# Wil-Lee/NN_BVH

Measured on AMD Instinct MI355X. Metric: Mray/s (closest-hit + any-hit), higher is better.
Workload: dtype f32; 1 GPU; crown, 1000x1400: one wavefront pass of 8 spp per step (8 spp per GPU-film) — primary, bounce-1 and bounce-2 closest-hit, shadow any-hit towards the light quads (batches pre-generated, hence independent: ONE launch; the dependent form is dependent_step), rays in --ray-order tile (a caller-side order the reference's integrator does not form: ray_order_probe), RecordShadowRayResult + RGBFilm::AddSam; sample_sets=4, geometry=procedural stand-in for crown (3548192 tris; data/crown.npz absent), tree=sah, triangles=3548192, nodes=7032259, rays_primary=11200000, rays_bounce=7410327, rays_bounce2=4392209, parallelism=tile-sharded x1, BVH replicated, film all-gather after the pass

## Files before the change

### nn_bvh_amd/aggregate.py

```python
import ctypes

import numpy as np

from . import _lib
from ._lib import HIT_DTYPE, NODE_DTYPE, PRIM_DTYPE, RAY_DTYPE, NNBVHError, check, ptr

SPLIT_METHODS = {"sah": 0, "hlbvh": 1, "middle": 2, "equal": 3}


def make_prims(tri_indices=None, patch_indices=None):
    nt = 0 if tri_indices is None else len(tri_indices)
    npch = 0 if patch_indices is None else len(patch_indices)
    prims = np.zeros(nt + npch, PRIM_DTYPE)
    prims["id"] = np.arange(nt + npch, dtype=np.int32)
    if nt:
        prims["kind"][:nt] = 0
        prims["v"][:nt, :3] = np.asarray(tri_indices, np.int32).reshape(nt, 3)
    if npch:
        prims["kind"][nt:] = 1
        prims["v"][nt:] = np.asarray(patch_indices, np.int32).reshape(npch, 4)
    return prims


def make_rays(o, d, tmax=np.inf, time=0.0):
# ... 206 lines not shown
                self._h = L.nnbvh_scene_create_instanced_animated(
                    ptr(self.nodes), len(self.nodes), int(n_top_nodes), ptr(self.ordered_prims),
                    len(self.ordered_prims), ptr(self.verts), len(self.verts), ptr(self.instances),
                    len(self.instances), ptr(self.animated), self.device)
            else:
                self._h = L.nnbvh_scene_create_instanced(
                    ptr(self.nodes), len(self.nodes), int(n_top_nodes), ptr(self.ordered_prims),
                    len(self.ordered_prims), ptr(self.verts), len(self.verts), ptr(self.instances),
                    len(self.instances), self.device)
        elif prim_alpha is not None:
            self.normals = None if normals is None else np.ascontiguousarray(normals, np.float32).reshape(-1, 3)
            self.prim_alpha = np.ascontiguousarray(prim_alpha, np.float32).reshape(-1)
            self.uvs = None if uvs is None else np.ascontiguousarray(uvs, np.float32).reshape(-1, 2)
            assert len(self.prim_alpha) == len(self.ordered_prims)
            assert self.normals is None or len(self.normals) == len(self.verts)
            assert self.uvs is None or len(self.uvs) == len(self.verts)
            self._h = L.nnbvh_scene_create_with_attributes(
                ptr(self.nodes), len(self.nodes), ptr(self.ordered_prims), len(self.ordered_prims), ptr(self.verts),
                ptr(self.normals) if self.normals is not None else None,
                ptr(self.uvs) if self.uvs is not None else None, ptr(self.prim_alpha), len(self.verts), self.device)
        elif normals is not None:
            self.normals = np.ascontiguousarray(normals, np.float32).reshape(-1, 3)
            assert len(self.normals) == len(self.verts)
            self._h = L.nnbvh_scene_create_with_normals(ptr(self.nodes), len(self.nodes), ptr(self.ordered_prims),
                                                        len(self.ordered_prims), ptr(self.verts), ptr(self.normals),
                                                        len(self.verts), self.device)
        else:
            self._h = L.nnbvh_scene_create(ptr(self.nodes), len(self.nodes), ptr(self.ordered_prims),
                                           len(self.ordered_prims), ptr(self.verts), len(self.verts),
                                           self.device)
        if not self._h:
            raise NNBVHError("nnbvh_scene_create: " + _lib.last_error())
        self._read_info()

    def close(self):
        if getattr(self, "_h", None):
            _lib.lib().nnbvh_scene_destroy(self._h)
            self._h = None

    def __del__(self):
        try:
            self.close()
        except Exception:
            pass

    def set_option(self, key, value):
        check(_lib.lib().nnbvh_scene_set_option(self._h, key.encode(), int(value)),
              f"set_option({key})")

    def sched_stats(self, reset=True):
        out = np.zeros(16, np.uint64)
        check(_lib.lib().nnbvh_scene_sched_stats(self._h, ptr(out), int(reset)), "sched_stats")
        return dict(zip(("int_trips", "int_lanes", "prim_trips", "prim_lanes", "refill_trips",
                         "refill_lanes", "i_nint", "i_nprim", "i_nidle", "spare0", "int_cycles",
                         "prim_cycles", "refill_cycles", "spare1", "int_steps", "int_step_lanes"),
                        (int(x) for x in out)))

    def Bounds(self):
        out = np.zeros(6, np.float32)
        check(_lib.lib().nnbvh_scene_bounds(self._h, ptr(out)), "nnbvh_scene_bounds")
        return out[:3].copy(), out[3:].copy()

    def Intersect(self, rays, out=None):
        rays = np.ascontiguousarray(rays, RAY_DTYPE)
        hits = np.zeros(len(rays), HIT_DTYPE) if out is None else out
        assert hits.dtype == HIT_DTYPE and len(hits) == len(rays) and hits.flags.c_contiguous
        check(_lib.lib().nnbvh_intersect_closest(self._h, ptr(rays), len(rays), ptr(hits)),
              "nnbvh_intersect_closest")
        return hits

    def IntersectP(self, rays, counts=False):
        rays = np.ascontiguousarray(rays, RAY_DTYPE)
        occ = np.zeros(len(rays), np.uint8)
        if counts:
            vis = np.zeros(len(rays), np.int32)
            tst = np.zeros(len(rays), np.int32)
            check(_lib.lib().nnbvh_intersect_any(self._h, ptr(rays), len(rays), ptr(occ),
                                                 ptr(vis), ptr(tst)), "nnbvh_intersect_any")
            return occ, vis, tst
        check(_lib.lib().nnbvh_intersect_any(self._h, ptr(rays), len(rays), ptr(occ), None, None),
              "nnbvh_intersect_any")
        return occ

    def intersect_device(self, d_rays, d_hits, n, stream=0):
        check(_lib.lib().nnbvh_intersect_closest_device(self._h, d_rays, n, d_hits, stream),
              "nnbvh_intersect_closest_device")

    def trace_batches_device(self, batches, stream=0):
        arr = np.zeros(len(batches), _lib.BATCH_DTYPE)
        for i, b in enumerate(batches):
            arr[i]["kind"] = {"closest": 0, "any": 1}[b[0]]
            arr[i]["d_rays"], arr[i]["n"], arr[i]["d_out"] = b[1], b[2], b[3]
            if len(b) > 4:
                arr[i]["d_nodes_visited"], arr[i]["d_prim_tests"] = b[4] or 0, b[5] or 0
        check(_lib.lib().nnbvh_trace_batches_device(self._h, ptr(arr), len(arr), stream),
              "nnbvh_trace_batches_device")

    def trace_batches_candidates_device(self, batches, candidates, stream=0):
        assert len(candidates) == len(batches)
        arr = np.zeros(len(batches), _lib.BATCH_DTYPE)
        for i, b in enumerate(batches):
            arr[i]["kind"] = {"closest": 0, "any": 1}[b[0]]
            arr[i]["d_rays"], arr[i]["n"], arr[i]["d_out"] = b[1], b[2], b[3]
            if len(b) > 4:
                arr[i]["d_nodes_visited"], arr[i]["d_prim_tests"] = b[4] or 0, b[5] or 0
        cs = (_lib.HostCandidates * max(len(batches), 1))()
        for i, c in enumerate(candidates):
            if c is not None:
# ... 121 lines not shown
```

### nn_bvh_amd/csrc/bvh_capi.cpp

```cpp
#include <algorithm>
#include <cmath>
#include <cstring>
#include <limits>
#include <vector>

#include "bvh_build_gpu.h"
#include "capi_internal.h"

namespace nnbvh {

static thread_local std::string g_error;
void set_error(const std::string &msg) { g_error = msg; }

}

using namespace nnbvh;

static bool validate_tree(const nnbvh_linear_node *nodes, int root, int n_tree, const nnbvh_prim *prims,
                          int n_prims, bool allow_instances, std::vector<uint8_t> &covered,
                          std::vector<uint8_t> &leaf_last, int *depth_out) {
    if (n_tree < 1) {
        set_error("scene_create: tree has no nodes");
        return false;
    }
// ... 653 lines not shown
        return NNBVH_ERR_ARG;
    }
    std::memset(out, 0, 16 * sizeof(uint64_t));
    if (!s->d_stats) return NNBVH_OK;
    DeviceGuard guard(s->device);
    if (!guard.ok) return NNBVH_ERR_DEVICE;
    if (!hip_ok(hipDeviceSynchronize(), "scene_sched_stats") ||
        !hip_ok(hipMemcpy(out, s->d_stats, 16 * sizeof(uint64_t), hipMemcpyDeviceToHost),
                "scene_sched_stats"))
        return NNBVH_ERR_DEVICE;
    if (reset) (void)hipMemset(s->d_stats, 0, 16 * sizeof(unsigned long long));
    return NNBVH_OK;
}

int nnbvh_scene_set_option(nnbvh_scene *s, const char *key, int value) {
    if (!s || !key) {
        set_error("set_option: null argument");
        return NNBVH_ERR_ARG;
    }
    std::lock_guard<std::mutex> lock(s->mu);
    std::string k(key);
    if (k == "stack_window") {
        if (value != 4 && value != 8 && value != 16) {
            set_error("set_option: stack_window must be 4, 8 or 16");
            return NNBVH_ERR_ARG;
        }
        s->window = value;
    } else if (k == "blocks_per_cu") {
        if (value < 0 || value > 8) {
            set_error("set_option: blocks_per_cu must be 0..8");
            return NNBVH_ERR_ARG;
        }
        s->blocks_per_cu = value;
    } else if (k == "int_repeat") {
        if (value < 1 || value > 16) {
            set_error("set_option: int_repeat must be 1..16");
            return NNBVH_ERR_ARG;
        }
        s->int_repeat = value;
    } else if (k == "host_chunk") {
        if (value < 1024) {
            set_error("set_option: host_chunk must be at least 1024 rays");
            return NNBVH_ERR_ARG;
        }
        s->host_chunk = value;
    } else if (k == "prim_repeat") {
        if (value < 1 || value > 16) {
            set_error("set_option: prim_repeat must be 1..16");
            return NNBVH_ERR_ARG;
        }
        s->prim_repeat = value;
    } else if (k == "fused_batches") {
        s->fused_batches = value ? 1 : 0;
    } else if (k == "xcd_queues") {
        s->xcd_queues = value ? 1 : 0;
    } else if (k == "prim_weight") {
        if (value < 1 || value > 64) {
            set_error("set_option: prim_weight must be 1..64");
            return NNBVH_ERR_ARG;
        }
        s->prim_weight = value;
    } else if (k == "refill_weight") {
        if (value < 1 || value > 64) {
            set_error("set_option: refill_weight must be 1..64");
            return NNBVH_ERR_ARG;
        }
        s->refill_weight = value;
    } else {
        set_error("set_option: unknown key");
        return NNBVH_ERR_ARG;
    }
    return NNBVH_OK;
}

}

Workspace *nnbvh::workspace_for(nnbvh_scene *s, hipStream_t stream) {
    auto it = s->workspaces.find(stream);
    if (it != s->workspaces.end()) return &it->second;
    Workspace w;
    const size_t spill_bytes = (size_t)std::max(s->depth - 2, 1) * (size_t)s->max_grid_threads * sizeof(uint2);
    if (!hip_ok(hipMalloc((void **)&w.queue, kMaxFusedBatches * kMaxQueues * kQueueStrideWords * sizeof(unsigned)),
                "hipMalloc(queue)"))
        return nullptr;
    if (!hip_ok(hipMalloc((void **)&w.spill, spill_bytes), "hipMalloc(spill)")) {
        (void)hipFree(w.queue);
        return nullptr;
    }
    return &(s->workspaces[stream] = w);
}
```

### nn_bvh_amd/csrc/bvh_trace.h

```cpp
#pragma once
#include <hip/hip_runtime.h>
#include <stdint.h>

#include "../../include/nnbvh.h"
#include "nnbvh_internal.h"

namespace nnbvh {

constexpr int kBlockThreads = 256;
constexpr int kMaxQueues = 8;
constexpr int kQueueStrideWords = 32;
constexpr int kMaxFusedBatches = 4;
constexpr int kFusedIndexBits = 28;

struct TraceParams {
    const float4 *wide;
    const float4 *prims;
    float rootMin[3], rootMax[3];
    int rootRef;
    const nnbvh_ray *rays;
    nnbvh_hit *hits;
    uint8_t *occluded;
    int32_t *visitedOut;
    int32_t *testsOut;
    long n;
    const int32_t *nDev;
    unsigned *queue;
    int nQueues;
    int primWeight;
    int refillWeight;
    int hasHostPrims;
    int intRepeat;
    int primRepeat;
    int fits32;
    unsigned long long *stats;
    uint2 *spill;
    const float *anim;
    int nBatches;
    unsigned anyMask;
    const nnbvh_ray *bRays[kMaxFusedBatches];
    void *bOut[kMaxFusedBatches];
    long bN[kMaxFusedBatches];
    const int32_t *bNDev[kMaxFusedBatches];
    nnbvh_ray_soa soa;
    nnbvh_ray_soa bSoa[kMaxFusedBatches];
    int hcCap;
    int32_t *hcCount;
    int32_t *hcBefore;
    int32_t *hcPrim;
    int32_t *hcInst;
    int bHcCap[kMaxFusedBatches];
    int32_t *bHcCount[kMaxFusedBatches];
    int32_t *bHcBefore[kMaxFusedBatches];
    int32_t *bHcPrim[kMaxFusedBatches];
    int32_t *bHcInst[kMaxFusedBatches];
};

hipError_t launch_zero_queue(unsigned *queue, int words, hipStream_t stream);
hipError_t launch_zero_words(int32_t *words, long n, int maxBlocks, hipStream_t stream);

hipError_t launch_trace(int mode, const TraceParams &p, int window, int instanced, int patches, int blocks,
                        hipStream_t stream, int *occupancy);

}
```

### nn_bvh_amd/csrc/bvh_trace.hip

```cpp
#include <hip/hip_runtime.h>
#include <stdint.h>

#include "bvh_trace.h"
#include "anim_math.h"
#include "spawn_math.h"
#include "stream_access.h"
#include "trace_math.h"

namespace nnbvh {

constexpr int kDone = (int)0x80000000;
constexpr int kReturn = (int)0x80000001;
constexpr int kEnter = (int)0x80000002;

#ifndef NNBVH_MINW_CLOSEST
#define NNBVH_MINW_CLOSEST 6
#endif
#ifndef NNBVH_MINW_ANY
#define NNBVH_MINW_ANY 6
#endif
#ifndef NNBVH_LEAN_EXTRA_WAVES
#define NNBVH_LEAN_EXTRA_WAVES 2
#endif
#ifndef NNBVH_MINW_ALPHA
// ... 16 lines not shown
void trace_kernel(TraceParams p) {
    static_assert(PATCH || !INST, "two-level scenes need the ray direction");
    static_assert(PATCH || !ALPHA, "the alpha test hashes the ray direction");
    static_assert(!HOSTC || (PATCH && (MODE == 0 || MODE == 2 || (MODE == 3 && !ALPHA && W == 8)) && !SOA),
                  "candidate mode: general instances of modes 0 / 2 / 3");
    __shared__ float s_stack[kBlockThreads / 64][W][2][64];
    constexpr bool kLean = !PATCH && !INST;
    constexpr int kColdRi = 0, kColdD = 1, kColdHit = kLean ? 0 : (PATCH ? 4 : 1),
                  kColdHost = kColdHit + ((MODE == 0 || MODE == 3) ? 4 : 0);
    constexpr int kColdBase = kColdHost + (kLean ? 0 : 1);
    constexpr int kSaveO = kColdBase, kSaveInv = kColdBase + 3, kSaveShear = kColdBase + 6,
                  kSaveKz = kColdBase + 9, kSaveTmax = kColdBase + 10, kSaveD = kColdBase + 11,
                  kResume = kColdBase + 14, kCurInst = kColdBase + 15, kHitInst = kColdBase + 16,
                  kInnerHit = kColdBase + 17, kColdTime = kColdBase + 18, kPendSlot = kColdBase + 19;
    constexpr int kColdFields = kColdBase + (INST ? 20 : 0);
    __shared__ float s_cold[kBlockThreads / 64][kColdFields > 0 ? kColdFields : 1][64];

    const int lane = threadIdx.x & 63;
    const int wave = threadIdx.x >> 6;
    const int gtid = blockIdx.x * kBlockThreads + threadIdx.x;
    float(*stk)[2][64] = s_stack[wave];
    float(*cold)[64] = s_cold[wave];
    int riReg = -1;
    if (!kLean) cold[kColdRi][lane] = __int_as_float(-1);
    const long spillStride = (long)gridDim.x * kBlockThreads;

    int q = 0;
    if (p.nQueues > 1) {
        unsigned xcc;
        asm volatile("s_getreg_b32 %0, hwreg(HW_REG_XCC_ID)" : "=s"(xcc));
        q = (int)(xcc & 0xf) % p.nQueues;
    }
    int queuesTried = 0;
    int curBatch = 0;
    long nRays = p.n;
    if (p.nDev) {
        const long nd = (long)*p.nDev;
        nRays = nd < 0 ? 0 : (nd < nRays ? nd : nRays);
    }

#ifdef NNBVH_STATS
    unsigned long long st[16] = {0, 0, 0, 0, 0, 0, 0, 0, 0, 0, 0, 0, 0, 0, 0, 0};
    unsigned long long stPrev = __builtin_amdgcn_s_memtime();
    int stKind = 2;
#endif
    RayState r;
    RayMasks masks = {0ull, 0ull, 0ull, 0ull, 0ull, 0ull};
    float tMax = 0.0f;
    int visited = 0, tests = 0;
    int cur = kDone, sp = 0, base = 0;
    int floor = -1;
    bool found = false;
    bool exhausted = false;

    auto pop_entry = [&](int &ref, float &key) {
        --sp;
        ref = __float_as_int(stk[sp & (W - 1)][0][lane]);
        key = stk[sp & (W - 1)][1][lane];
        asm volatile("" : "+v"(ref), "+v"(key));
        if (sp < base) {
            const uint2 e = p.spill[(long)sp * spillStride + gtid];
            base = sp;
            ref = (int)e.x;
            key = __uint_as_float(e.y);
            asm volatile("" : "+v"(ref), "+v"(key));
        }
        if (MODE != 2) visited += 1;
    };
    auto pop_next = [&]() -> int {
        const int lowest = (INST && floor > 0) ? floor : 0;
        const int none = (INST && floor >= 0) ? kReturn : kDone;
        if (sp <= lowest) return none;
        int ref;
        float key;
        pop_entry(ref, key);
        if (key < tMax) return ref;
        while (sp > lowest) {
            pop_entry(ref, key);
            if (key < tMax) return ref;
        }
        return none;
    };

    auto enter_instance = [&](int slot, unsigned flags, float4 s0, float4 s1, float4 s2) {
        const float4 s3 = p.prims[slot + 3], s4 = p.prims[slot + 4], s5 = p.prims[slot + 5];
        const V3 dOuter = {cold[kColdD][lane], cold[kColdD + 1][lane], cold[kColdD + 2][lane]};
        cold[kSaveO][lane] = r.o.x;
        cold[kSaveO + 1][lane] = r.o.y;
        cold[kSaveO + 2][lane] = r.o.z;
        cold[kSaveInv][lane] = r.inv.x;
        cold[kSaveInv + 1][lane] = r.inv.y;
        cold[kSaveInv + 2][lane] = r.inv.z;
        cold[kSaveShear][lane] = r.sx;
        cold[kSaveShear + 1][lane] = r.sy;
        cold[kSaveShear + 2][lane] = r.sz;
        cold[kSaveKz][lane] = __int_as_float(r.kz);
        cold[kSaveTmax][lane] = tMax;
        cold[kSaveD][lane] = dOuter.x;
        cold[kSaveD + 1][lane] = dOuter.y;
        cold[kSaveD + 2][lane] = dOuter.z;
        cold[kResume][lane] = __int_as_float((flags & kPrimLast) ? kDone : ~(slot + 6));
        cold[kCurInst][lane] = __int_as_float(__float_as_int(s0.w) + 1);
        cold[kInnerHit][lane] = 0.0f;
        V3 oIn, dIn;
        float4 m0 = s2, m1 = s3, m2 = s4;
        if (INST == 2 && (flags & kPrimAnimated) && p.anim)
// ... 172 lines not shown
                            pick_batch(p.bHcBefore, tag >> kFusedIndexBits)[tag & ((1 << kFusedIndexBits) - 1)] = c;
                        }
                    }
                } else {
                    found = true;
                }
            }
            if (MODE != 0 && found) cur = kDone;
            else if (flags & kPrimLast) cur = pop_next();
            else cur = ~next;
        }
    };

    auto interior_math = [&](const float4 q0, const float4 q1, const float4 q2, const float4 q3) {
        const int ref0 = __float_as_int(q3.x), ref1 = __float_as_int(q3.y);
        const int axis = __float_as_int(q3.z);
        const bool swap = ((r.kz >> axis) & 1) != 0;
        const float k0 = kLean ? slab_entry_key(q0.x, q0.y, q0.z, q0.w, q1.x, q1.y, r, masks)
                               : slab_entry_key(q0.x, q0.y, q0.z, q0.w, q1.x, q1.y, r);
        const float k1 = kLean ? slab_entry_key(q1.z, q1.w, q2.x, q2.y, q2.z, q2.w, r, masks)
                               : slab_entry_key(q1.z, q1.w, q2.x, q2.y, q2.z, q2.w, r);
        const int nearRef = swap ? ref1 : ref0, farRef = swap ? ref0 : ref1;
        const float nearT = swap ? k1 : k0, farT = swap ? k0 : k1;
        visited += 1;
        const bool doPush = (MODE == 1) || (farT < __builtin_inff());
        if (doPush && sp - base == W - 1) {
            uint2 e;
            e.x = __float_as_uint(stk[base & (W - 1)][0][lane]);
            e.y = __float_as_uint(stk[base & (W - 1)][1][lane]);
            p.spill[(long)base * spillStride + gtid] = e;
            ++base;
        }
        stk[sp & (W - 1)][0][lane] = __int_as_float(farRef);
        stk[sp & (W - 1)][1][lane] = farT;
        sp += doPush ? 1 : 0;
        if (MODE == 0 || MODE == 3) visited += doPush ? 0 : 1;
        cur = nearT < tMax ? nearRef : pop_next();
    };
    auto interior_step = [&]() {
#ifdef NNBVH_STATS
        st[14] += 1;
        st[15] += __popcll(__ballot(cur >= 0));
#endif
        if (cur >= 0) {
            const float4 *rec = kLean ? reinterpret_cast<const float4 *>(reinterpret_cast<const char *>(p.wide) + ((unsigned)cur << 6))
                                      : p.wide + 4 * (long)cur;
            const float4 q3 = rec[3];
            const float4 q0 = rec[0], q1 = rec[1], q2 = rec[2];
            interior_math(q0, q1, q2, q3);
        }
    };

    for (;;) {
#ifdef NNBVH_STATS
        {
            const unsigned long long now = __builtin_amdgcn_s_memtime();
            st[10 + stKind] += now - stPrev;
            stPrev = now;
        }
#endif
        const bool isInt = cur >= 0;
        const bool isIdle = cur == kDone;
        const int nInt = __popcll(__ballot(isInt));
        const unsigned long long idleMask = __ballot(isIdle);
        const int nIdle = __popcll(idleMask);
        const int nEnter = (INST == 2 && NNBVH_ANIM_ENTER_WEIGHT > 0) ? __popcll(__ballot(cur == kEnter)) : 0;
        const int nPrim = 64 - nInt - nIdle - nEnter;

        const int sI = nInt * 16, sP = nPrim * p.primWeight;
        const int sR = exhausted ? 0 : nIdle * p.refillWeight;
#ifdef NNBVH_STATS
        unsigned long long &stTrips = (nIdle == 64 || (sR > sI && sR > sP)) ? st[4]
                                      : ((sP > sI || nInt == 0) ? st[2] : st[0]);
        (&stTrips)[0] += 1;
        (&stTrips)[1] += (nIdle == 64 || (sR > sI && sR > sP)) ? nIdle
                         : ((sP > sI || nInt == 0) ? nPrim : nInt);
        stKind = (&stTrips == &st[4]) ? 2 : ((&stTrips == &st[2]) ? 1 : 0);
        if (&stTrips == &st[0]) {
            st[6] += nInt;
            st[7] += nPrim;
            st[8] += nIdle;
        }
#endif
        if (nIdle == 64 || (sR > sI && sR > sP)) {
            const int ri = isIdle ? (kLean ? riReg : __float_as_int(cold[kColdRi][lane])) : -1;
            if constexpr (MODE == 3 && HOSTC) {
                if (ri >= 0) {
                    const int b = ri >> kFusedIndexBits;
                    const long idx = ri & ((1 << kFusedIndexBits) - 1);
                    void *outp = pick_batch(p.bOut, b);
                    const int c = __float_as_int(cold[kColdHost][lane]);
                    if (pick_batch(p.bHcCap, b) > 0) pick_batch(p.bHcCount, b)[idx] = c;
                    if ((p.anyMask >> b) & 1u) {
                        store_stream(reinterpret_cast<uint8_t *>(outp) + idx, (uint8_t)(found ? 1 : (c != 0 ? 2 : 0)));
                    } else {
                        float4 h0, h1;
                        h0.x = cold[kColdHit][lane];
                        h0.y = tMax;
                        h0.z = cold[kColdHit + 1][lane];
                        h0.w = cold[kColdHit + 2][lane];
                        h1.x = cold[kColdHit + 3][lane];
                        h1.y = __int_as_float(visited);
                        h1.z = __int_as_float(tests);
                        h1.w = INST ? cold[kHitInst][lane] : 0.0f;
                        if (c < 0) h1.w = __int_as_float(-1);
                        float4 *out = reinterpret_cast<float4 *>(outp) + 2 * idx;
                        store_stream(out, h0);
                        store_stream(out + 1, h1);
                    }
                }
// ... 97 lines not shown
            if (isIdle) {
                const int tag = (MODE == 3 && newRi >= 0) ? (newRi | (curBatch << kFusedIndexBits)) : newRi;
                if (kLean) riReg = tag;
                else cold[kColdRi][lane] = __int_as_float(tag);
            }
            if (newRi >= 0) {
                const nnbvh_ray *batchRays = MODE == 3 ? p.bRays[curBatch] : p.rays;
                float4 r0, r1;
                if (!SOA || batchRays) {
                    const float4 *in = reinterpret_cast<const float4 *>(batchRays) + 2 * (long)newRi;
                    r0 = load_stream(in);
                    r1 = load_stream(in + 1);
                } else {
                    const nnbvh_ray_soa &q = MODE == 3 ? p.bSoa[curBatch] : p.soa;
                    auto ld = [&](const float *a) { return load_stream(a + newRi); };
                    r0 = {ld(q.ox), ld(q.oy), ld(q.oz), q.tmax ? ld(q.tmax) : __builtin_inff()};
                    r1 = {ld(q.dx), ld(q.dy), ld(q.dz), q.time ? ld(q.time) : 0.0f};
                }
                r.o = {r0.x, r0.y, r0.z};
                tMax = r0.w;
                const V3 d = {r1.x, r1.y, r1.z};
                if (PATCH) {
                    cold[kColdD][lane] = d.x;
                    cold[kColdD + 1][lane] = d.y;
                    cold[kColdD + 2][lane] = d.z;
                }
                r.inv = {1.0f / d.x, 1.0f / d.y, 1.0f / d.z};
                ray_shear(r, d);
                if (MODE == 0 || MODE == 3) {
                    cold[kColdHit][lane] = __int_as_float(-1);
                    cold[kColdHit + 1][lane] = 0.0f;
                    cold[kColdHit + 2][lane] = 0.0f;
                    cold[kColdHit + 3][lane] = 0.0f;
                }
                if (INST) {
                    cold[kHitInst][lane] = 0.0f;
                    cold[kCurInst][lane] = 0.0f;
                    cold[kColdTime][lane] = r1.w;
                    floor = -1;
                }
                if (!kLean && (HOSTC || p.hasHostPrims)) cold[kColdHost][lane] = 0.0f;
                visited = 1;
                tests = 0;
                found = false;
                sp = base = 0;
                float tEntry;
                const bool rootHit =
                    slab_partial(p.rootMin[0], p.rootMin[1], p.rootMin[2], p.rootMax[0],
                                 p.rootMax[1], p.rootMax[2], r, tEntry) &&
                    (tEntry < tMax);
                cur = rootHit ? p.rootRef : kDone;
            }
            if (kLean) masks = ray_masks(r);
            continue;
        }

        if (INST == 2 && NNBVH_ANIM_ENTER_WEIGHT > 0 && nEnter > 0 &&
            ((nInt == 0 && nPrim == 0) || (nEnter * NNBVH_ANIM_ENTER_WEIGHT > sI && nEnter * NNBVH_ANIM_ENTER_WEIGHT > sP))) {
            if (cur == kEnter) {
                const int slot = __float_as_int(cold[kPendSlot][lane]);
                const float4 s0 = p.prims[slot], s1 = p.prims[slot + 1], s2 = p.prims[slot + 2];
                enter_instance(slot, __float_as_uint(s1.w), s0, s1, s2);
            }
            continue;
        }

        if (sP > sI || nInt == 0) {
            const int nPrep = (MODE == 3) ? 1 : p.primRepeat;
            int prep = 0;
            do {
            if (cur < 0 && cur != kDone) {
                if (INST && cur == kReturn) leave_instance();
                if (cur < 0 && cur != kDone && cur != kReturn && (INST != 2 || cur != kEnter)) {
                    const int slot = ~cur;
                    const float4 *pr = kLean ? reinterpret_cast<const float4 *>(reinterpret_cast<const char *>(p.prims) + ((unsigned)slot << 4))
                                             : p.prims + slot;
                    float4 s0 = pr[0], s1 = pr[1], s2 = pr[2];
                    asm volatile("" : "+v"(s0.x), "+v"(s0.y), "+v"(s0.z), "+v"(s0.w), "+v"(s1.x), "+v"(s1.y),
                                      "+v"(s1.z), "+v"(s1.w), "+v"(s2.x), "+v"(s2.y), "+v"(s2.z), "+v"(s2.w));
                    prim_math(slot, s0, s1, s2);
                }
            }
            } while (++prep < nPrep && __ballot(cur < 0 && cur != kDone) != 0ull);
        } else {
            if (MODE == 3) {
                interior_step();
                if (p.intRepeat > 1 && __ballot(cur >= 0) != 0ull) {
                    interior_step();
                    if (p.intRepeat > 2 && __ballot(cur >= 0) != 0ull) {
                        interior_step();
                        for (int rep = 3; rep < p.intRepeat && __ballot(cur >= 0) != 0ull; ++rep) interior_step();
                    }
                }
            } else {
            int rep = 0;
            do {
                interior_step();
            } while (++rep < p.intRepeat && __ballot(cur >= 0) != 0ull);
            }
        }
    }
#ifdef NNBVH_STATS
    if (lane == 0 && p.stats)
        for (int k = 0; k < 16; ++k) atomicAdd(&p.stats[k], st[k]);
#endif
}

template <int MODE, int W, int INST, int PATCH, int ALPHA = 0, int SOA = 0, int HOSTC = 0>
static hipError_t launch_one(const TraceParams &p, int blocks, hipStream_t stream, int *occupancy) {
    if (occupancy) {
        return hipOccupancyMaxActiveBlocksPerMultiprocessor(
            occupancy, trace_kernel<MODE, W, INST, PATCH, ALPHA, SOA, HOSTC>, kBlockThreads, 0);
    }
    hipLaunchKernelGGL((trace_kernel<MODE, W, INST, PATCH, ALPHA, SOA, HOSTC>), dim3((unsigned)blocks),
                       dim3(kBlockThreads), 0, stream, p);
    return hipGetLastError();
}

template <int MODE, int ALPHA, int HOSTC>
static hipError_t launch_inst(const TraceParams &p, int instanced, int blocks, hipStream_t stream, int *occupancy) {
    if (!instanced) return launch_one<MODE, 8, 0, 1, ALPHA, 0, HOSTC>(p, blocks, stream, occupancy);
    return p.anim ? launch_one<MODE, 8, 2, 1, ALPHA, 0, HOSTC>(p, blocks, stream, occupancy)
                  : launch_one<MODE, 8, 1, 1, ALPHA, 0, HOSTC>(p, blocks, stream, occupancy);
}
template <int MODE, int HOSTC>
static hipError_t launch_general(const TraceParams &p, int instanced, int patches, int blocks, hipStream_t stream,
                                 int *occupancy) {
    if (patches & 4) return launch_inst<MODE, 2, HOSTC>(p, instanced, blocks, stream, occupancy);
    if (patches & 2) return launch_inst<MODE, 1, HOSTC>(p, instanced, blocks, stream, occupancy);
    return launch_inst<MODE, 0, HOSTC>(p, instanced, blocks, stream, occupancy);
}

static hipError_t launch_fused(const TraceParams &p, int window, int instanced, int patches, int blocks,
                               hipStream_t stream, int *occupancy) {
    if (window != 8 || (patches & 2)) return hipErrorInvalidValue;
    if (p.hcCap > 0) {
        if (instanced) return p.anim ? launch_one<3, 8, 2, 1, 0, 0, 1>(p, blocks, stream, occupancy)
                                     : launch_one<3, 8, 1, 1, 0, 0, 1>(p, blocks, stream, occupancy);
        return launch_one<3, 8, 0, 1, 0, 0, 1>(p, blocks, stream, occupancy);
    }
    if (instanced) return p.anim ? launch_one<3, 8, 2, 1>(p, blocks, stream, occupancy)
                                 : launch_one<3, 8, 1, 1>(p, blocks, stream, occupancy);
    bool soa = false;
    for (int b = 0; b < p.nBatches; ++b) soa = soa || !p.bRays[b];
    if (!patches && !p.hasHostPrims && p.fits32)
        return soa ? launch_one<3, 8, 0, 0, 0, 1>(p, blocks, stream, occupancy) : launch_one<3, 8, 0, 0>(p, blocks, stream, occupancy);
    if (soa) return hipErrorInvalidValue;
    return launch_one<3, 8, 0, 1>(p, blocks, stream, occupancy);
}

template <int MODE>
static hipError_t launch_mode(const TraceParams &p, int window, int instanced, int patches, int blocks,
                              hipStream_t stream, int *occupancy) {
    if constexpr (MODE == 0 || MODE == 2) {
// ... 48 lines not shown
```

### nn_bvh_amd/csrc/capi_internal.h

```cpp
#pragma once
#include <hip/hip_runtime.h>

#include <cstddef>
#include <cstdint>
#include <map>
#include <mutex>
#include <string>

#include "bvh_trace.h"
#include "interaction.h"

namespace nnbvh {

inline bool hip_ok(hipError_t e, const char *what) {
    if (e == hipSuccess) return true;
    set_error(std::string(what) + ": " + hipGetErrorString(e));
    return false;
}

struct DeviceGuard {
    int prev = -1;
    bool ok = false;
    explicit DeviceGuard(int dev) {
        if (hipGetDevice(&prev) != hipSuccess) prev = -1;
        ok = hip_ok(hipSetDevice(dev), "hipSetDevice");
    }
    ~DeviceGuard() {
        if (prev >= 0) (void)hipSetDevice(prev);
    }
};

struct Workspace {
    unsigned *queue = nullptr;
    uint2 *spill = nullptr;
    void *d_in = nullptr, *d_out = nullptr, *d_aux0 = nullptr, *d_aux1 = nullptr;
    size_t in_bytes = 0, out_bytes = 0, aux_bytes = 0;
    void *d_hits = nullptr;
    size_t hits_bytes = 0;
    static constexpr int kScratch = 12;
    void *scratch[kScratch] = {nullptr, nullptr, nullptr, nullptr, nullptr, nullptr, nullptr, nullptr, nullptr, nullptr, nullptr, nullptr};
    size_t scratch_bytes[kScratch] = {0, 0, 0, 0, 0, 0, 0, 0, 0, 0, 0, 0};
};

struct HostSlot {
    hipEvent_t ev_in = nullptr, ev_traced = nullptr, ev_out = nullptr;
    void *d_in = nullptr, *h_in = nullptr;
    size_t d_in_bytes = 0, h_in_bytes = 0;
    void *d_out[3] = {nullptr, nullptr, nullptr}, *h_out[3] = {nullptr, nullptr, nullptr};
    size_t d_out_bytes[3] = {0, 0, 0}, h_out_bytes[3] = {0, 0, 0};
};

}

struct nnbvh_scene {
    int device = 0;
    int n_cus = 0;
    int n_interior = 0;
    int64_t n_slots = 0;
    int depth = 0;
    float bounds[6];
    int root_ref = 0;
    float4 *d_wide = nullptr;
    float4 *d_prims = nullptr;
    float *d_anim = nullptr;
    int n_anim = 0;
    size_t device_bytes = 0;
    int window = 8;
    int blocks_per_cu = 0;
    int xcd_queues = 1;
    int prim_weight = 32;
    int refill_weight = 8;
    unsigned long long *d_stats = nullptr;
    int instanced = 0;
    int has_host_prims = 0;
    int has_patches = 1;
    int has_alpha = 0;
    int fused_batches = 1;
    int int_repeat = 3;
    int prim_repeat = 2;
    int max_grid_threads = 0;
    double build_ms[1] = {0};
    std::mutex mu;
    std::map<hipStream_t, nnbvh::Workspace> workspaces;
    static constexpr int kHostSlots = 3, kHostChunks = 6;
    nnbvh::HostSlot host_slots[kHostSlots];
    hipStream_t host_up = nullptr, host_trace = nullptr, host_down = nullptr;
    int64_t host_chunk = 1 << 20;
    static constexpr int kSideStreams = 4;
    hipStream_t side[kSideStreams] = {nullptr, nullptr, nullptr, nullptr};
    hipEvent_t ev_fork = nullptr;
    hipEvent_t ev_join[kSideStreams] = {nullptr, nullptr, nullptr, nullptr};
};

struct nnbvh_shading_mesh {
    int device = 0;
    int n_cus = 0;
    nnbvh::ShadingMeshDevice d;
};

namespace nnbvh {

Workspace *workspace_for(nnbvh_scene *s, hipStream_t stream);

void fill_anim_entry(const nnbvh_animated_transform &a, float *t);

struct SceneCall {
    DeviceGuard guard;
    std::unique_lock<std::mutex> lock;
    Workspace *w = nullptr;
    bool good;
    explicit SceneCall(nnbvh_scene *s) : guard(s->device), good(guard.ok) {
        if (good) lock = std::unique_lock<std::mutex>(s->mu);
    }
    SceneCall(nnbvh_scene *s, hipStream_t stream) : SceneCall(s) {
        if (good) good = (w = workspace_for(s, stream)) != nullptr;
    }
    bool ok() const { return good; }
};

inline bool grow(void **ptr, size_t *have, size_t need, const char *what) {
    if (*have >= need) return true;
    if (*ptr) (void)hipFree(*ptr);
    *ptr = nullptr;
    *have = 0;
    if (!hip_ok(hipMalloc(ptr, need), what)) return false;
    *have = need;
    return true;
}

inline int patch_bits(const nnbvh_scene *s) { return s->has_patches + 2 * (s->has_alpha != 0) + 4 * (s->has_alpha == 2); }
// ... 35 lines not shown
```

### nn_bvh_amd/csrc/capi_trace.cpp

```cpp
#include <algorithm>
#include <cstring>
#include <thread>

#include "capi_internal.h"

using namespace nnbvh;

int nnbvh::grid_blocks(nnbvh_scene *s, int mode, int candidates) {
    int per_cu = s->blocks_per_cu;
    if (per_cu <= 0) {
        TraceParams dummy{};
        dummy.hasHostPrims = s->has_host_prims;
        dummy.anim = s->d_anim;
        dummy.fits32 = scene_fits32(s);
        dummy.hcCap = candidates;
        int occ = 0;
        if (launch_trace(mode, dummy, s->window, s->instanced, patch_bits(s), 0, nullptr, &occ) != hipSuccess ||
            occ <= 0)
            occ = std::max(1, std::min(8, 160 / (s->window * 2)));
        per_cu = occ;
    }
    per_cu = std::min(per_cu, 8);
    return s->n_cus * per_cu;
}

bool nnbvh::zero_candidates(const nnbvh_scene *s, const nnbvh_host_candidates *hc, int64_t n, bool closest,
                            hipStream_t stream) {
    return hip_ok(launch_zero_words(hc->count, (long)n, s->n_cus * 8, stream), "candidate count reset launch") &&
           (!closest || !hc->before ||
            hip_ok(launch_zero_words(hc->before, (long)n, s->n_cus * 8, stream), "candidate before reset launch"));
}

static TraceParams scene_params(const nnbvh_scene *s, const Workspace *w) {
    TraceParams p{};
    p.wide = s->d_wide;
    p.prims = s->d_prims;
    std::memcpy(p.rootMin, s->bounds, 12);
    std::memcpy(p.rootMax, s->bounds + 3, 12);
    p.rootRef = s->root_ref;
    p.queue = w->queue;
    p.nQueues = s->xcd_queues ? kMaxQueues : 1;
    p.primWeight = s->prim_weight;
    p.refillWeight = s->refill_weight;
    p.stats = s->d_stats;
    p.intRepeat = s->int_repeat;
    p.primRepeat = s->prim_repeat;
    p.fits32 = scene_fits32(s);
    p.hasHostPrims = s->has_host_prims;
    p.spill = w->spill;
    p.anim = s->d_anim;
    return p;
}

static int run_trace(nnbvh_scene *s, hipStream_t stream, int mode, const TraceParams &p, int queue_words,
                     const char *what) {
    if (!hip_ok(launch_zero_queue(p.queue, queue_words, stream), "queue reset launch")) return NNBVH_ERR_DEVICE;
    int blocks = grid_blocks(s, mode, p.hcCap);
    const int64_t need = (p.n + kBlockThreads - 1) / kBlockThreads;
    if (need < blocks) blocks = (int)std::max<int64_t>(need, 1);
    if (!hip_ok(launch_trace(mode, p, s->window, s->instanced, patch_bits(s), blocks, stream, nullptr), what))
        return NNBVH_ERR_DEVICE;
    return NNBVH_OK;
}

int nnbvh::launch(nnbvh_scene *s, Workspace *w, hipStream_t stream, const TraceJob &job) {
    TraceParams p = scene_params(s, w);
    if (job.soa) p.soa = *job.soa;
    p.rays = (const nnbvh_ray *)job.rays;
    p.hits = (nnbvh_hit *)job.hits;
    p.occluded = (uint8_t *)job.occluded;
    p.visitedOut = (int32_t *)job.visited;
    p.testsOut = (int32_t *)job.tests;
    p.n = (long)job.n;
    p.nDev = job.d_n;
    if (const nnbvh_host_candidates *hc = job.hc) {
        int32_t *before = job.mode == 0 ? hc->before : nullptr;
        const size_t bytes = (size_t)job.n * sizeof(int32_t);
        if (!job.hc_zeroed &&
            (!hip_ok(hipMemsetAsync(hc->count, 0, bytes, stream), "hipMemsetAsync(count)") ||
             (before && !hip_ok(hipMemsetAsync(before, 0, bytes, stream), "hipMemsetAsync(before)"))))
            return NNBVH_ERR_DEVICE;
        if (s->has_host_prims) {
            p.hcCap = hc->capacity;
            p.hcCount = hc->count;
            p.hcBefore = before;
            p.hcPrim = hc->prim;
            p.hcInst = hc->instance;
        }
    }
    return run_trace(s, stream, job.mode, p, kMaxQueues * kQueueStrideWords, "trace kernel launch");
}

int nnbvh::launch_fused_batches(nnbvh_scene *s, Workspace *w, hipStream_t stream, const nnbvh_batch *batches,
                                int n_batches, const int32_t *const *d_n, const nnbvh_ray_soa *const *soas,
                                const nnbvh_host_candidates *cands) {
    TraceParams p = scene_params(s, w);
    int64_t total = 0;
    for (int i = 0; i < n_batches; ++i) {
        if (batches[i].n == 0) continue;
        const int b = p.nBatches++;
        p.bRays[b] = (const nnbvh_ray *)batches[i].d_rays;
        p.bOut[b] = batches[i].d_out;
        p.bN[b] = (long)batches[i].n;
        p.bNDev[b] = d_n ? d_n[i] : nullptr;
        if (soas && soas[i]) p.bSoa[b] = *soas[i];
        if (batches[i].kind == NNBVH_BATCH_ANY) p.anyMask |= 1u << b;
        total += batches[i].n;
        if (cands && cands[i].capacity > 0) {
            const bool closest = batches[i].kind == NNBVH_BATCH_CLOSEST;
            if (!zero_candidates(s, &cands[i], batches[i].n, closest, stream)) return NNBVH_ERR_DEVICE;
            if (s->has_host_prims) {
                p.hcCap = 1;
                p.bHcCap[b] = cands[i].capacity;
                p.bHcCount[b] = cands[i].count;
                p.bHcBefore[b] = closest ? cands[i].before : nullptr;
                p.bHcPrim[b] = cands[i].prim;
                p.bHcInst[b] = cands[i].instance;
            }
        }
    }
    if (p.nBatches == 0) return NNBVH_OK;
    p.n = (long)total;
    return run_trace(s, stream, 3, p, kMaxFusedBatches * kMaxQueues * kQueueStrideWords, "fused trace kernel launch");
}

bool nnbvh::batches_fusable(const nnbvh_scene *s, const nnbvh_batch *batches, int n_batches) {
    bool fusable = s->fused_batches && n_batches <= kMaxFusedBatches && s->window == 8 && !s->has_alpha;
    for (int i = 0; fusable && i < n_batches; ++i)
        fusable = batches[i].n < (1LL << kFusedIndexBits) &&
                  !(batches[i].kind == NNBVH_BATCH_ANY && (batches[i].d_nodes_visited || batches[i].d_prim_tests));
    return fusable;
}

const char *nnbvh::candidates_fault(const nnbvh_host_candidates *c, bool closest) {
    if (!c) return "candidates is NULL";
    if (c->capacity < 1 || c->capacity > 16) return "capacity must be 1..16";
    if (!c->count || !c->prim || !c->instance) return "count, prim and instance are required";
    if (closest && !c->before) return "before is required for closest hit";
    return nullptr;
}

bool nnbvh::candidates_ok(const char *fn, const nnbvh_host_candidates *c, bool closest) {
    const char *why = candidates_fault(c, closest);
    if (why) set_error(std::string(fn) + ": " + why);
    return !why;
}

static bool batch_args_ok(const char *fn, const nnbvh_scene *s, int64_t n, const void *rays, const void *out,
                          const char *candidates_wrong = nullptr) {
    const char *why = nullptr;
    if (!s || n < 0 || (n > 0 && (!rays || !out))) why = "bad argument";
    else if (candidates_wrong) why = candidates_wrong;
    else if (n >= 0x7fffffffLL) why = "at most 2^31-1 rays per call";
    if (why) set_error(std::string(fn) + ": " + why);
    return !why;
}

extern "C" {

int nnbvh_intersect_closest_device(nnbvh_scene *s, const void *d_rays, int64_t n, void *d_hits,
                                   void *stream) {
    if (!batch_args_ok("intersect_closest_device", s, n, d_rays, d_hits)) return NNBVH_ERR_ARG;
    if (n == 0) return NNBVH_OK;
    SceneCall call(s, (hipStream_t)stream);
    if (!call.ok()) return NNBVH_ERR_DEVICE;
    return launch(s, call.w, (hipStream_t)stream, {.mode = 0, .rays = d_rays, .n = n, .hits = d_hits});
}

int nnbvh_intersect_any_device(nnbvh_scene *s, const void *d_rays, int64_t n, void *d_occluded,
                               void *d_nodes_visited, void *d_prim_tests, void *stream) {
    if (!batch_args_ok("intersect_any_device", s, n, d_rays, d_occluded)) return NNBVH_ERR_ARG;
    if (n == 0) return NNBVH_OK;
    SceneCall call(s, (hipStream_t)stream);
    if (!call.ok()) return NNBVH_ERR_DEVICE;
// ... 364 lines not shown
```

Baseline: 4789 Mray/s.

## Split traversal stacks of remaining any-hit rays onto idle lanes during drain

In the fused multi-batch kernel, once a wave's ray queue is exhausted it enters a drain loop. Idle lanes take pending stack entries from lanes still tracing any-hit rays and trace those subtrees as helpers, sharing the occlusion result through a per-lane scratch word. Any-hit batches are also reordered to run last so that the tail is made of shadow rays, which can be split this way. The change aims to cut low SIMD utilisation in the wave tail, at the cost of cross-lane shuffles, extra registers and more complex control flow.

```diff
diff --git a/nn_bvh_amd/aggregate.py b/nn_bvh_amd/aggregate.py
--- a/nn_bvh_amd/aggregate.py
+++ b/nn_bvh_amd/aggregate.py
@@ -282,8 +282,8 @@
         out = np.zeros(16, np.uint64)
         check(_lib.lib().nnbvh_scene_sched_stats(self._h, ptr(out), int(reset)), "sched_stats")
         return dict(zip(("int_trips", "int_lanes", "prim_trips", "prim_lanes", "refill_trips",
-                         "refill_lanes", "i_nint", "i_nprim", "i_nidle", "spare0", "int_cycles",
-                         "prim_cycles", "refill_cycles", "spare1", "int_steps", "int_step_lanes"),
+                         "refill_lanes", "i_nint", "i_nprim", "i_nidle", "wave_cycles", "int_cycles",
+                         "prim_cycles", "refill_cycles", "drain_cycles", "int_steps", "int_step_lanes"),
                         (int(x) for x in out)))
 
     def Bounds(self):
diff --git a/nn_bvh_amd/csrc/bvh_capi.cpp b/nn_bvh_amd/csrc/bvh_capi.cpp
--- a/nn_bvh_amd/csrc/bvh_capi.cpp
+++ b/nn_bvh_amd/csrc/bvh_capi.cpp
@@ -729,6 +729,8 @@
         s->prim_repeat = value;
     } else if (k == "fused_batches") {
         s->fused_batches = value ? 1 : 0;
+    } else if (k == "drain_split") {
+        s->drain_split = value ? 1 : 0;
     } else if (k == "xcd_queues") {
         s->xcd_queues = value ? 1 : 0;
     } else if (k == "prim_weight") {
diff --git a/nn_bvh_amd/csrc/bvh_trace.h b/nn_bvh_amd/csrc/bvh_trace.h
--- a/nn_bvh_amd/csrc/bvh_trace.h
+++ b/nn_bvh_amd/csrc/bvh_trace.h
@@ -12,6 +12,7 @@
 constexpr int kQueueStrideWords = 32;
 constexpr int kMaxFusedBatches = 4;
 constexpr int kFusedIndexBits = 28;
+constexpr int kHelperBatch = 7;
 
 struct TraceParams {
     const float4 *wide;
@@ -54,6 +55,7 @@
     int32_t *bHcBefore[kMaxFusedBatches];
     int32_t *bHcPrim[kMaxFusedBatches];
     int32_t *bHcInst[kMaxFusedBatches];
+    int drainSplit;
 };
 
 hipError_t launch_zero_queue(unsigned *queue, int words, hipStream_t stream);
diff --git a/nn_bvh_amd/csrc/bvh_trace.hip b/nn_bvh_amd/csrc/bvh_trace.hip
--- a/nn_bvh_amd/csrc/bvh_trace.hip
+++ b/nn_bvh_amd/csrc/bvh_trace.hip
@@ -92,6 +92,8 @@
     int floor = -1;
     bool found = false;
     bool exhausted = false;
+    constexpr bool kSplit = kLean && MODE == 3;
+    bool drain = false;
 
     auto pop_entry = [&](int &ref, float &key) {
         --sp;
@@ -370,10 +372,13 @@
     };
 
     for (;;) {
+        if (kSplit && drain) break;
 #ifdef NNBVH_STATS
         {
             const unsigned long long now = __builtin_amdgcn_s_memtime();
             st[10 + stKind] += now - stPrev;
+            st[9] += now - stPrev;
+            if (exhausted) st[13] += now - stPrev;
             stPrev = now;
         }
 #endif
@@ -577,6 +582,9 @@
                 cur = rootHit ? p.rootRef : kDone;
             }
             if (kLean) masks = ray_masks(r);
+            if constexpr (kSplit) {
+                drain = exhausted && p.drainSplit;
+            }
             continue;
         }
 
@@ -625,6 +633,119 @@
             }
         }
     }
+
+    if constexpr (kSplit) {
+        if (drain) {
+            constexpr int kHelperTag = kHelperBatch << kFusedIndexBits;
+            float *const myWord = &cold[kColdHit + 1][lane];
+            auto lane_now = [&]() {
+                int l;
+                asm volatile("v_mbcnt_lo_u32_b32 %0, -1, 0\n\tv_mbcnt_hi_u32_b32 %0, -1, %0" : "=v"(l));
+                return l;
+            };
+            auto rank_in = [&](unsigned long long m) {
+                return (int)__builtin_amdgcn_mbcnt_hi((unsigned)(m >> 32), __builtin_amdgcn_mbcnt_lo((unsigned)m, 0u));
+            };
+            for (;;) {
+                const bool helper = riReg >= kHelperTag;
+                const int self = lane_now();
+                const int owner = helper ? riReg - kHelperTag : self;
+                float *word = myWord + (owner - self);
+                const bool occl = riReg >= 0 && ((p.anyMask >> (riReg >> kFusedIndexBits)) & 1u) != 0;
+                if (occl && found) *word = 1.0f;
+                __builtin_amdgcn_wave_barrier();
+                const bool hitSeen = occl && *word != 0.0f;
+                if (hitSeen) cur = kDone;
+                const bool allIdle = __ballot(cur != kDone) == 0ull;
+                if (riReg >= 0 && !helper && cur == kDone && (!occl || hitSeen || allIdle)) {
+                    const int b = riReg >> kFusedIndexBits;
+                    const long idx = riReg & ((1 << kFusedIndexBits) - 1);
+                    void *outp = pick_batch(p.bOut, b);
+                    if (occl) {
+                        store_stream(reinterpret_cast<uint8_t *>(outp) + idx, (uint8_t)((found || hitSeen) ? 1 : 0));
+                    } else {
+                        int32_t *out = reinterpret_cast<int32_t *>(outp) + 8 * idx;
+                        store_stream(out, (int32_t)__float_as_int(cold[kColdHit][lane]));
+                        store_stream(out + 1, (int32_t)__float_as_int(tMax));
+                        store_stream(out + 2, (int32_t)__float_as_int(cold[kColdHit + 1][lane]));
+                        store_stream(out + 3, (int32_t)__float_as_int(cold[kColdHit + 2][lane]));
+                        store_stream(out + 4, (int32_t)__float_as_int(cold[kColdHit + 3][lane]));
+                        store_stream(out + 5, (int32_t)visited);
+                        store_stream(out + 6, (int32_t)tests);
+                        store_stream(out + 7, (int32_t)0);
+                    }
+                    riReg = -1;
+                }
+                if (helper && cur == kDone) riReg = -1;
+                if (allIdle) break;
+
+                const bool isFree = riReg == -1;
+                const bool canGive = occl && cur != kDone && sp > 0;
+                const unsigned long long freeMask = __ballot(isFree), giveMask = __ballot(canGive);
+                if (freeMask != 0ull && giveMask != 0ull) {
+                    int give = kDone;
+                    if (canGive && rank_in(giveMask) < __popcll(freeMask)) give = pop_next();
+                    int src = self;
+                    for (unsigned long long fm = freeMask, gm = giveMask; fm != 0ull && gm != 0ull; fm &= fm - 1ull, gm &= gm - 1ull)
+                        src = self == __builtin_ctzll(fm) ? __builtin_ctzll(gm) : src;
+                    const bool take = src != self;
+                    const int from = src << 2;
+                    const int gRef = __builtin_amdgcn_ds_bpermute(from, give);
+                    const bool accept = take && gRef != kDone;
+                    auto pull = [&](int &v) {
+                        const int g = __builtin_amdgcn_ds_bpermute(from, v);
+                        v = accept ? g : v;
+                    };
+                    auto pullf = [&](float &v) {
+                        const float g = __int_as_float(__builtin_amdgcn_ds_bpermute(from, __float_as_int(v)));
+                        v = accept ? g : v;
+                    };
+                    int own = owner;
+                    pull(own);
+                    pull(r.kz);
+                    pullf(tMax);
+                    pullf(r.o.x);
+                    pullf(r.o.y);
+                    asm volatile("" : "+v"(r.o.z), "+v"(r.inv.x), "+v"(r.inv.y), "+v"(r.inv.z)
+                                 : "v"(own), "v"(r.kz), "v"(tMax), "v"(r.o.x), "v"(r.o.y));
+                    pullf(r.o.z);
+                    pullf(r.inv.x);
+                    pullf(r.inv.y);
+                    pullf(r.inv.z);
+                    asm volatile("" : "+v"(r.sx), "+v"(r.sy), "+v"(r.sz) : "v"(r.o.z), "v"(r.inv.x), "v"(r.inv.y), "v"(r.inv.z));
+                    pullf(r.sx);
+                    pullf(r.sy);
+                    pullf(r.sz);
+                    if (accept) {
+                        cur = gRef;
+                        sp = base = 0;
+                        found = false;
+                        riReg = kHelperTag | own;
+                    }
+                }
+                masks = ray_masks(r);
+
+                if (__ballot(cur >= 0) != 0ull) interior_step();
+                if (__ballot(cur < 0 && cur != kDone) != 0ull) {
+                    if (cur < 0 && cur != kDone) {
+                        const int slot = ~cur;
+                        const float4 *pr = reinterpret_cast<const float4 *>(reinterpret_cast<const char *>(p.prims) + ((unsigned)slot << 4));
+                        float4 s0 = pr[0], s1 = pr[1], s2 = pr[2];
+                        asm volatile("" : "+v"(s0.x), "+v"(s0.y), "+v"(s0.z), "+v"(s0.w), "+v"(s1.x), "+v"(s1.y),
+                                          "+v"(s1.z), "+v"(s1.w), "+v"(s2.x), "+v"(s2.y), "+v"(s2.z), "+v"(s2.w));
+                        prim_math(slot, s0, s1, s2);
+                    }
+                }
+            }
+#ifdef NNBVH_STATS
+            {
+                const unsigned long long now = __builtin_amdgcn_s_memtime();
+                st[9] += now - stPrev;
+                st[13] += now - stPrev;
+            }
+#endif
+        }
+    }
 #ifdef NNBVH_STATS
     if (lane == 0 && p.stats)
         for (int k = 0; k < 16; ++k) atomicAdd(&p.stats[k], st[k]);
diff --git a/nn_bvh_amd/csrc/capi_internal.h b/nn_bvh_amd/csrc/capi_internal.h
--- a/nn_bvh_amd/csrc/capi_internal.h
+++ b/nn_bvh_amd/csrc/capi_internal.h
@@ -76,6 +76,7 @@
     int has_patches = 1;
     int has_alpha = 0;
     int fused_batches = 1;
+    int drain_split = 1;
     int int_repeat = 3;
     int prim_repeat = 2;
     int max_grid_threads = 0;
diff --git a/nn_bvh_amd/csrc/capi_trace.cpp b/nn_bvh_amd/csrc/capi_trace.cpp
--- a/nn_bvh_amd/csrc/capi_trace.cpp
+++ b/nn_bvh_amd/csrc/capi_trace.cpp
@@ -49,6 +49,7 @@
     p.hasHostPrims = s->has_host_prims;
     p.spill = w->spill;
     p.anim = s->d_anim;
+    p.drainSplit = s->drain_split;
     return p;
 }
 
@@ -96,8 +97,15 @@
                                 const nnbvh_host_candidates *cands) {
     TraceParams p = scene_params(s, w);
     int64_t total = 0;
-    for (int i = 0; i < n_batches; ++i) {
-        if (batches[i].n == 0) continue;
+    int order[kMaxFusedBatches], n_order = 0;
+    for (int pass = 0; pass < 2; ++pass)
+        for (int i = 0; i < n_batches; ++i) {
+            if (batches[i].n == 0) continue;
+            const bool last = s->drain_split && batches[i].kind == NNBVH_BATCH_ANY;
+            if (last == (pass == 1)) order[n_order++] = i;
+        }
+    for (int k = 0; k < n_order; ++k) {
+        const int i = order[k];
         const int b = p.nBatches++;
         p.bRays[b] = (const nnbvh_ray *)batches[i].d_rays;
         p.bOut[b] = batches[i].d_out;
@@ -120,6 +128,7 @@
         }
     }
     if (p.nBatches == 0) return NNBVH_OK;
+    p.anyMask |= 1u << kHelperBatch;
     p.n = (long)total;
     return run_trace(s, stream, 3, p, kMaxFusedBatches * kMaxQueues * kQueueStrideWords, "fused trace kernel launch");
 }
```

New measurement: 4735 Mray/s. -1.1%, worse.
